# ade-ma/LibRedio

Measured on NVIDIA B200. Metric: Msamples/s cf32 through FIR-decimate+FFT chain, higher is better.
Workload: dtype f32

## Files before the change

libredio_b200/csrc/common.cuh:

```cuda
#pragma once
#include <cuda_runtime.h>
#include <cstdint>
#include <cstdio>
#include <cstdarg>
#include <cstring>
#include <cstdlib>
#include <new>
#include "../../include/libredio_cuda.h"

struct lrc_ctx {
    int          device;
    int          n_sm;
    cudaStream_t stream;
    cudaStream_t copy_stream;
    cudaStream_t out_stream;
    int          numa_node;
    int          numa_nodes;
};

void lrc_set_error(const char *fmt, ...);

#define LRC_CUDA(call)                                                                       \
    do {                                                                                     \
        cudaError_t e__ = (call);                                                            \
        if (e__ != cudaSuccess) {                                                            \
            lrc_set_error("%s:%d %s -> %s", __FILE__, __LINE__, #call, cudaGetErrorString(e__)); \
            return LRC_ERR_CUDA;                                                             \
        }                                                                                    \
    } while (0)

#define LRC_REQUIRE(cond, code, msg)                                                         \
    do {                                                                                     \
        if (!(cond)) {                                                                       \
            lrc_set_error("%s:%d %s", __FILE__, __LINE__, msg);                              \
            return (code);                                                                   \
        }                                                                                    \
    } while (0)

static inline cudaStream_t lrc_stream(const lrc_ctx *ctx, void *s)
{
    return s ? reinterpret_cast<cudaStream_t>(s) : ctx->stream;
}

#define LRC_BIND(ctx)                                                                        \
    do {                                                                                     \
        LRC_REQUIRE((ctx) != nullptr, LRC_ERR_INVALID, "null context");                      \
        LRC_CUDA(cudaSetDevice((ctx)->device));                                              \
    } while (0)

static inline size_t ceil_div(size_t a, size_t b) { return (a + b - 1) / b; }

static inline size_t lrc_grid_mult(const char *env_name, size_t dflt)
{
    const char *e = getenv(env_name);
    if (!e) return dflt;
    const long v = atol(e);
    return v > 0 ? (size_t)v : dflt;
}

#ifdef __CUDACC__

__device__ __forceinline__ uint64_t pk2(float lo, float hi)
{
    uint64_t r;
    asm("mov.b64 %0, {%1, %2};" : "=l"(r) : "f"(lo), "f"(hi));
    return r;
}
__device__ __forceinline__ float2 upk2(uint64_t v)
{
    float2 r;
    asm("mov.b64 {%0, %1}, %2;" : "=f"(r.x), "=f"(r.y) : "l"(v));
    return r;
}
__device__ __forceinline__ float2 add2(float2 a, float2 b)
{
    uint64_t r;
    asm("add.rn.f32x2 %0, %1, %2;" : "=l"(r) : "l"(pk2(a.x, a.y)), "l"(pk2(b.x, b.y)));
    return upk2(r);
}
__device__ __forceinline__ float2 sub2(float2 a, float2 b)
{
    uint64_t r;
    asm("sub.rn.f32x2 %0, %1, %2;" : "=l"(r) : "l"(pk2(a.x, a.y)), "l"(pk2(b.x, b.y)));
    return upk2(r);
}
__device__ __forceinline__ float2 mul2(float2 a, float2 b)
{
    uint64_t r;
    asm("mul.rn.f32x2 %0, %1, %2;" : "=l"(r) : "l"(pk2(a.x, a.y)), "l"(pk2(b.x, b.y)));
    return upk2(r);
}
__device__ __forceinline__ float2 fma2(float2 a, float2 b, float2 c)
{
    uint64_t r;
    asm("fma.rn.f32x2 %0, %1, %2, %3;" : "=l"(r) : "l"(pk2(a.x, a.y)), "l"(pk2(b.x, b.y)), "l"(pk2(c.x, c.y)));
    return upk2(r);
}

__device__ __forceinline__ float2 cmulf(float2 a, float2 b)
{
    return fma2(a, make_float2(b.x, b.x), mul2(make_float2(a.y, a.x), make_float2(-b.y, b.y)));
}
__device__ __forceinline__ float2 cmul_conjb(float2 a, float2 b)
{
    return fma2(a, make_float2(b.x, b.x), mul2(make_float2(a.y, a.x), make_float2(b.y, -b.y)));
}

__device__ __forceinline__ float4 ldg_stream_f4(const float4 *p)
{
    float4 r;
    asm volatile("ld.global.nc.L1::no_allocate.v4.f32 {%0, %1, %2, %3}, [%4];"
                 : "=f"(r.x), "=f"(r.y), "=f"(r.z), "=f"(r.w) : "l"(p));
    return r;
}
__device__ __forceinline__ uint4 ldg_stream_u4(const uint4 *p)
{
    uint4 r;
    asm volatile("ld.global.nc.L1::no_allocate.v4.u32 {%0, %1, %2, %3}, [%4];"
                 : "=r"(r.x), "=r"(r.y), "=r"(r.z), "=r"(r.w) : "l"(p));
    return r;
}
__device__ __forceinline__ void stg_stream_f4(float4 *p, float4 v)
{
    asm volatile("st.global.L1::no_allocate.v4.f32 [%0], {%1, %2, %3, %4};"
                 :: "l"(p), "f"(v.x), "f"(v.y), "f"(v.z), "f"(v.w) : "memory");
}

__device__ __forceinline__ uint32_t smem_u32(const void *p)
{
    return static_cast<uint32_t>(__cvta_generic_to_shared(p));
}

__device__ __forceinline__ void mbar_init(uint64_t *bar, uint32_t count)
{
    asm volatile("mbarrier.init.shared::cta.b64 [%0], %1;" :: "r"(smem_u32(bar)), "r"(count));
}
__device__ __forceinline__ void mbar_fence_init()
{
    asm volatile("fence.mbarrier_init.release.cluster;" ::: "memory");
}
__device__ __forceinline__ void mbar_expect_tx(uint64_t *bar, uint32_t bytes)
{
    asm volatile("mbarrier.arrive.expect_tx.shared::cta.b64 _, [%0], %1;"
                 :: "r"(smem_u32(bar)), "r"(bytes) : "memory");
}
__device__ __forceinline__ void mbar_wait(uint64_t *bar, uint32_t parity)
{
    asm volatile(
        "{\n"
        ".reg .pred p;\n"
        "WAIT_%=:\n"
        "mbarrier.try_wait.parity.shared::cta.b64 p, [%0], %1;\n"
        "@p bra DONE_%=;\n"
        "bra WAIT_%=;\n"
        "DONE_%=:\n"
        "}\n" :: "r"(smem_u32(bar)), "r"(parity) : "memory");
}
__device__ __forceinline__ void tma_load_1d(void *smem_dst, const void *gmem_src, uint32_t bytes,
                                            uint64_t *bar)
{
    asm volatile(
        "cp.async.bulk.shared::cluster.global.mbarrier::complete_tx::bytes [%0], [%1], %2, [%3];"
        :: "r"(smem_u32(smem_dst)), "l"(gmem_src), "r"(bytes), "r"(smem_u32(bar)) : "memory");
}
__device__ __forceinline__ void tma_load_1d_evict_first(void *smem_dst, const void *gmem_src,
                                                        uint32_t bytes, uint64_t *bar)
{
    uint64_t pol;
    asm volatile("createpolicy.fractional.L2::evict_first.b64 %0, 1.0;" : "=l"(pol));
    asm volatile(
        "cp.async.bulk.shared::cluster.global.mbarrier::complete_tx::bytes.L2::cache_hint [%0], [%1], %2, [%3], %4;"
        :: "r"(smem_u32(smem_dst)), "l"(gmem_src), "r"(bytes), "r"(smem_u32(bar)), "l"(pol) : "memory");
}
__device__ __forceinline__ void cp_async4(void *smem_dst, const void *gmem_src, uint32_t src_bytes)
{
    asm volatile("cp.async.ca.shared.global [%0], [%1], 4, %2;" :: "r"(smem_u32(smem_dst)), "l"(gmem_src), "r"(src_bytes) : "memory");
}
__device__ __forceinline__ void cp_async_commit()
{
    asm volatile("cp.async.commit_group;" ::: "memory");
}
template <int N>
__device__ __forceinline__ void cp_async_wait_group()
{
    asm volatile("cp.async.wait_group %0;" :: "n"(N) : "memory");
}
__device__ __forceinline__ void fence_proxy_async()
{
    asm volatile("fence.proxy.async.shared::cta;" ::: "memory");
}
__device__ __forceinline__ void named_bar_sync(int id, int nthreads)
{
    asm volatile("bar.sync %0, %1;" :: "r"(id), "r"(nthreads) : "memory");
}

__device__ __forceinline__ void named_bar_arrive(int id, int nthreads)
{
    asm volatile("bar.arrive %0, %1;" :: "r"(id), "r"(nthreads) : "memory");
}

#endif
```

libredio_b200/csrc/k_chain.cu:

```cuda
#include "fir_core.cuh"
#include "fft_core.cuh"
#include "unpack.cuh"
#include "chain_generic.cuh"
#include <vector>
#include <cmath>

using namespace lrfft;

int    lrc_make_twiddles(int nfft, float2 **d_tw);
int    lrc_log2_exact(int n);
size_t lrc_psd_frames_per_item(size_t k_avg);
int    lrc_psd_ensure_partial(float **d_partial, size_t *cap, size_t need_floats);
int    lrc_psd_reduce(const float *d_partial, float *d_rows, int nfft, size_t ipr, size_t n_rows, float scale,
                      int accumulate, cudaStream_t s);

struct lrc_chain {
    lrc_ctx *ctx;
    int      ntaps, decim, nfft, log2n, window;
    bool     fused;
    bool     fused_generic;
    std::vector<float> taps;
    float2  *d_tw;
    float   *d_win;
    float   *d_partial; size_t partial_cap;
    lrc_fir *fir; lrc_psd *psd;
    float   *d_tmp; size_t tmp_cap;
    float   *d_ring[2]; size_t ring_cap;
    uint8_t *d_ring_u8[2]; size_t ring_u8_cap;
    cudaEvent_t ev_ready[2], ev_free[2];
    float   *d_rows; size_t rows_cap;
    float   *d_u8tmp; size_t u8tmp_cap;
};

template <int NTAPS, int DECIM, int LOG2N, int R>
struct ChainCfg {
    using Tile = FirTile<NTAPS, DECIM, R>;
    using FFT = CtaFFT<LOG2N, false>;
    static constexpr int N = 1 << LOG2N;
    static constexpr int FRAME_ADV = N * DECIM;
    static constexpr int TILE_IN = (N - 1) * DECIM + NTAPS;
    static constexpr int NFIR = (N + R - 1) / R;
    static constexpr int NFIR_T = (NFIR + 31) / 32 * 32;
    static constexpr int NFFT_T = FFT::T;
    static constexpr int NT = NFIR_T + NFFT_T;
    static constexpr int TILE_SAMPLES = (NFIR - 1) * Tile::STEP + Tile::WIN;
    static constexpr uint32_t TMA_BYTES = TILE_IN * 8;
    static constexpr uint32_t RAW_BYTES = TILE_IN * 2;
    static constexpr uint32_t RAW_TMA_BYTES = RAW_BYTES & ~15u;
    static constexpr int RAW_WORDS = (RAW_BYTES + 3) / 4;
    static constexpr int RAW_OFF = (TILE_SAMPLES * 8 - (int)((RAW_BYTES + 15) & ~15u)) & ~15;
    static constexpr int RAW_PER_THREAD = (RAW_WORDS + NFIR_T - 1) / NFIR_T;
    static_assert(RAW_BYTES % 4 == 0, "whole words");
    static_assert((RAW_BYTES - RAW_TMA_BYTES) / 4 <= NFIR_T, "the rest words fall into the last two words of their owners");
    static constexpr int OFF_HAND = TILE_SAMPLES * 8;
    static constexpr int OFF_XCHG = OFF_HAND + FFT::SMEM_CPX * 8;
    static constexpr int OFF_BAR = OFF_XCHG + FFT::SMEM_CPX * 8;
    static constexpr int SMEM_BYTES = OFF_BAR + 16;
    static_assert(TMA_BYTES % 16 == 0 && (FRAME_ADV * 8) % 16 == 0, "TMA alignment");
    static_assert(NFFT_T % 32 == 0, "FFT threads must be whole warps");
};

enum { BAR_FULL = 1, BAR_EMPTY = 2, BAR_TILE = 3, BAR_FFT = 4 };

template <int NTAPS, int DECIM, int LOG2N, int R, bool IS_U8>
__global__ void __launch_bounds__(ChainCfg<NTAPS, DECIM, LOG2N, R>::NT, 2)
chain_kernel(const float2 *__restrict__ in, const float2 *__restrict__ tw, const float *__restrict__ win,
             float *__restrict__ partial, size_t k_avg, size_t fpi, size_t ipr, size_t n_items,
             const __grid_constant__ FirTaps<NTAPS> taps)
{
    using Cfg = ChainCfg<NTAPS, DECIM, LOG2N, R>;
    using Tile = typename Cfg::Tile;
    using FFT = typename Cfg::FFT;
    constexpr int N = Cfg::N, E = FFT::E, T = FFT::T;
    extern __shared__ __align__(128) uint8_t smem[];
    float2 *tile = reinterpret_cast<float2 *>(smem);
    float2 *hand = reinterpret_cast<float2 *>(smem + Cfg::OFF_HAND);
    float2 *xchg = reinterpret_cast<float2 *>(smem + Cfg::OFF_XCHG);
    uint64_t *bar = reinterpret_cast<uint64_t *>(smem + Cfg::OFF_BAR);
    const int tid = threadIdx.x;
    if (tid == 0) { mbar_init(bar, 1); mbar_fence_init(); }
    __syncthreads();
    if ((size_t)blockIdx.x >= n_items) return;

    auto item_range = [&](size_t item, size_t &f0, size_t &f1) {
        const size_t row = item / ipr, c = item % ipr;
        f0 = row * k_avg + c * fpi;
        f1 = f0 + fpi;
        if (f1 > (row + 1) * k_avg) f1 = (row + 1) * k_avg;
    };

    if (tid < Cfg::NFIR_T) {
        uint32_t phase = 0;
        bool first = true;
        size_t item = blockIdx.x, f0, f1;
        item_range(item, f0, f1);
        size_t f = f0;
        const uint8_t *in8 = reinterpret_cast<const uint8_t *>(in);
        uint8_t *raw = smem + Cfg::RAW_OFF;
        auto load_frame = [&](size_t fr) {
            if (IS_U8) {
                mbar_expect_tx(bar, Cfg::RAW_TMA_BYTES);
                tma_load_1d_evict_first(raw, in8 + fr * (size_t)Cfg::FRAME_ADV * 2, Cfg::RAW_TMA_BYTES, bar);
            } else {
                mbar_expect_tx(bar, Cfg::TMA_BYTES);
                tma_load_1d_evict_first(tile, in + fr * Cfg::FRAME_ADV, Cfg::TMA_BYTES, bar);
            }
        };
        if (tid == 0) load_frame(f);
        while (true) {
            if (IS_U8) {
                constexpr int TMA_WORDS = (int)(Cfg::RAW_TMA_BYTES / 4), KL = Cfg::RAW_PER_THREAD;
                uint32_t rest[2] = {0u, 0u};
#pragma unroll
                for (int k = KL - 2; k < KL; ++k) {
                    const int i = tid + k * Cfg::NFIR_T;
                    if (k >= 0 && i >= TMA_WORDS && i < Cfg::RAW_WORDS)
                        rest[k - (KL - 2)] = *reinterpret_cast<const uint32_t *>(in8 + f * (size_t)Cfg::FRAME_ADV * 2 + 4 * (size_t)i);
                }
                mbar_wait(bar, phase);
                uint32_t wv[Cfg::RAW_PER_THREAD];
                const uint32_t *rw = reinterpret_cast<const uint32_t *>(raw);
#pragma unroll
                for (int k = 0; k < KL; ++k) {
                    const int i = tid + k * Cfg::NFIR_T;
                    wv[k] = i < TMA_WORDS ? rw[i] : (k >= KL - 2 ? rest[k - (KL - 2)] : 0u);
                }
                named_bar_sync(BAR_TILE, Cfg::NFIR_T);
                float4 *t4 = reinterpret_cast<float4 *>(tile);
#pragma unroll
                for (int k = 0; k < Cfg::RAW_PER_THREAD; ++k) {
                    const int i = tid + k * Cfg::NFIR_T;
                    if (i < Cfg::RAW_WORDS)
                        t4[i] = make_float4(lr_i2f_byte(wv[k], 0), lr_i2f_byte(wv[k], 1), lr_i2f_byte(wv[k], 2), lr_i2f_byte(wv[k], 3));
                }
                named_bar_sync(BAR_TILE, Cfg::NFIR_T);
            } else {
                mbar_wait(bar, phase);
            }
            phase ^= 1;
            float2 acc[R];
            if (tid < Cfg::NFIR) Tile::run_cf32(tile + (size_t)tid * Tile::STEP, taps, acc);
            size_t nf = f + 1, nitem = item, nf1 = f1;
            if (nf == f1) {
                nitem = item + gridDim.x;
                if (nitem < n_items) item_range(nitem, nf, nf1);
            }
            const bool has_next = nitem < n_items;
            named_bar_sync(BAR_TILE, Cfg::NFIR_T);
            if (tid == 0 && has_next) load_frame(nf);
            if (!first) named_bar_sync(BAR_EMPTY, Cfg::NT);
            first = false;
            if (tid < Cfg::NFIR) {
#pragma unroll
                for (int r = 0; r < R; ++r) {
                    const int o = tid * R + r;
                    if (o < N) hand[FFT::pad(o)] = acc[r];
                }
            }
            __threadfence_block();
            named_bar_arrive(BAR_FULL, Cfg::NT);
            if (!has_next) break;
            item = nitem; f = nf; f1 = nf1;
        }
    } else {
        const int t = tid - Cfg::NFIR_T;
        float w[E], acc[E];
#pragma unroll
        for (int e = 0; e < E; ++e) { w[e] = win[t + e * T]; acc[e] = 0.f; }
        size_t item = blockIdx.x, f0, f1;
        item_range(item, f0, f1);
        size_t f = f0;
        while (true) {
            size_t nf = f + 1, nitem = item, nf1 = f1;
            if (nf == f1) {
                nitem = item + gridDim.x;
                if (nitem < n_items) item_range(nitem, nf, nf1);
            }
            const bool has_next = nitem < n_items;
            named_bar_sync(BAR_FULL, Cfg::NT);
            float2 v[E];
#pragma unroll
            for (int e = 0; e < E; ++e) {
                const float2 x = hand[FFT::pad(t + e * T)];
                v[e] = make_float2(x.x * w[e], x.y * w[e]);
            }
            if (has_next) named_bar_arrive(BAR_EMPTY, Cfg::NT);
            FFT::run(v, xchg, tw, t, SyncNamed{BAR_FFT, T});
#pragma unroll
            for (int e = 0; e < E; ++e) acc[e] = fmaf(v[e].x, v[e].x, fmaf(v[e].y, v[e].y, acc[e]));
            const bool item_done = (f + 1 == f1);
            if (item_done) {
                float *dst = partial + item * N + t;
#pragma unroll
                for (int e = 0; e < E; ++e) { dst[e * T] = acc[e]; acc[e] = 0.f; }
            }
            if (!has_next) break;
            item = nitem; f = nf; f1 = nf1;
        }
    }
}

static const size_t SEG_FRAMES = 400;

extern "C" int lrc_chain_create(lrc_ctx *ctx, const float *h_taps, int ntaps, int decim, int nfft, int window,
                                lrc_chain **out)
{
    LRC_BIND(ctx);
    LRC_REQUIRE(out && h_taps && ntaps >= 1 && decim >= 1, LRC_ERR_INVALID, "lrc_chain_create: bad arguments");
    const int l2 = lrc_log2_exact(nfft);
    if (l2 < 1 || l2 > 13) {
        lrc_set_error("lrc_chain_create: nfft=%d: only powers of two in [2, 8192]", nfft);
        return LRC_ERR_UNSUPPORTED;
    }
    lrc_chain *c = new (std::nothrow) lrc_chain();
    LRC_REQUIRE(c != nullptr, LRC_ERR_NOMEM, "out of host memory");
    c->ctx = ctx; c->ntaps = ntaps; c->decim = decim; c->nfft = nfft; c->log2n = l2; c->window = window;
    c->taps.assign(h_taps, h_taps + ntaps);
    c->fused = (ntaps == 64 && decim == 10 && nfft == 1024);
    c->fused_generic = false;
    if (!c->fused && !getenv("LRC_CHAIN_NO_GENERIC")) {
        c->fused_generic = lrc_chaing_has(ntaps, decim, l2, getenv("LRC_CHAIN_GENERIC_ALL") != nullptr);
    }
    c->d_tw = nullptr; c->d_win = nullptr; c->d_partial = nullptr; c->partial_cap = 0;
    c->fir = nullptr; c->psd = nullptr; c->d_tmp = nullptr; c->tmp_cap = 0;
    c->d_ring[0] = c->d_ring[1] = nullptr; c->ring_cap = 0; c->d_rows = nullptr; c->rows_cap = 0;
    c->d_ring_u8[0] = c->d_ring_u8[1] = nullptr; c->ring_u8_cap = 0;
    c->d_u8tmp = nullptr; c->u8tmp_cap = 0;
    c->ev_ready[0] = c->ev_ready[1] = c->ev_free[0] = c->ev_free[1] = nullptr;
    int rc = lrc_fir_create(ctx, h_taps, ntaps, decim, &c->fir);
    if (!rc) rc = lrc_psd_create(ctx, nfft, window, &c->psd);
    if (!rc) rc = lrc_make_twiddles(nfft, &c->d_tw);
    if (!rc) {
        std::vector<float> w(nfft);
        const double pi = 3.14159265358979323846264338327950288;
        for (int i = 0; i < nfft; ++i)
            w[i] = window == LRC_WINDOW_HANN ? (float)(0.5 - 0.5 * cos(2.0 * pi * i / nfft)) : 1.0f;
        if (cudaMalloc(&c->d_win, sizeof(float) * nfft) != cudaSuccess ||
            cudaMemcpy(c->d_win, w.data(), sizeof(float) * nfft, cudaMemcpyHostToDevice) != cudaSuccess) {
            lrc_set_error("lrc_chain_create: %s", cudaGetErrorString(cudaGetLastError()));
            rc = LRC_ERR_CUDA;
        }
    }
    if (rc) { lrc_chain_destroy(c); return rc; }
    *out = c;
    return LRC_OK;
}

extern "C" int lrc_chain_destroy(lrc_chain *c)
{
    if (!c) return LRC_OK;
    cudaSetDevice(c->ctx->device);
    lrc_fir_destroy(c->fir); lrc_psd_destroy(c->psd);
    cudaFree(c->d_tw); cudaFree(c->d_win); cudaFree(c->d_partial); cudaFree(c->d_tmp);
    cudaFree(c->d_ring[0]); cudaFree(c->d_ring[1]); cudaFree(c->d_rows);
    cudaFree(c->d_ring_u8[0]); cudaFree(c->d_ring_u8[1]); cudaFree(c->d_u8tmp);
    for (int i = 0; i < 2; ++i) {
        if (c->ev_ready[i]) cudaEventDestroy(c->ev_ready[i]);
        if (c->ev_free[i]) cudaEventDestroy(c->ev_free[i]);
    }
    delete c;
    return LRC_OK;
}

extern "C" size_t lrc_chain_frames(const lrc_chain *c, size_t n_in)
{
    if (!c) return 0;
    const size_t tile_in = (size_t)(c->nfft - 1) * c->decim + c->ntaps;
    if (n_in < tile_in) return 0;
    return (n_in - tile_in) / ((size_t)c->nfft * c->decim) + 1;
}

extern "C" int lrc_chain_kind(const lrc_chain *c)
{
    if (!c) return 0;
    return c->fused ? 1 : (c->fused_generic ? 2 : 0);
}

template <bool IS_U8>
static int chain_launch_fused(lrc_chain *c, const void *d_in, size_t k_local, size_t fpi, size_t ipr, size_t n_items, cudaStream_t s)
{
    using Cfg = ChainCfg<64, 10, 10, 7>;
    auto kern = chain_kernel<64, 10, 10, 7, IS_U8>;
    LRC_CUDA(cudaFuncSetAttribute(kern, cudaFuncAttributeMaxDynamicSharedMemorySize, Cfg::SMEM_BYTES));
    int occ = 1;
    LRC_CUDA(cudaOccupancyMaxActiveBlocksPerMultiprocessor(&occ, kern, Cfg::NT, Cfg::SMEM_BYTES));
    if (occ < 1) occ = 1;
    static const size_t gm = lrc_grid_mult("LRC_CHAIN_GRID", 1);
    size_t blocks = (size_t)c->ctx->n_sm * occ * gm;
    if (blocks > n_items) blocks = n_items;
    FirTaps<64> taps;
    for (int i = 0; i < 64; ++i) taps.h[i] = c->taps[i];
    kern<<<(unsigned)blocks, Cfg::NT, Cfg::SMEM_BYTES, s>>>((const float2 *)d_in, c->d_tw, c->d_win, c->d_partial,
                                                           k_local, fpi, ipr, n_items, taps);
    LRC_CUDA(cudaGetLastError());
    return LRC_OK;
}

static int chain_launch(lrc_chain *c, const void *d_in_any, int input_is_u8, size_t rows_local, size_t k_local, float *d_rows,
                        float scale, int accumulate, cudaStream_t s)
{
    const float *d_in = (const float *)d_in_any;
    if (rows_local == 0 || k_local == 0) return LRC_OK;
    const size_t fpi = lrc_psd_frames_per_item(k_local);
    const size_t ipr = ceil_div(k_local, fpi);
    const size_t n_items = rows_local * ipr;
    int rc = lrc_psd_ensure_partial(&c->d_partial, &c->partial_cap, n_items * (size_t)c->nfft);
    if (rc) return rc;
    if (c->fused) {
        rc = input_is_u8 ? chain_launch_fused<true>(c, d_in_any, k_local, fpi, ipr, n_items, s)
                         : chain_launch_fused<false>(c, d_in_any, k_local, fpi, ipr, n_items, s);
        if (rc) return rc;
        return lrc_psd_reduce(c->d_partial, d_rows, c->nfft, ipr, rows_local, scale, accumulate, s);
    }
    LRC_REQUIRE(!input_is_u8, LRC_ERR_INVALID, "chain_launch: u8 input without a fused instance");
    if (c->fused_generic) {
        chaing::Args a;
        a.in = (const float2 *)d_in_any; a.tw = c->d_tw; a.win = c->d_win; a.taps = c->taps.data(); a.partial = c->d_partial;
        a.k_avg = k_local; a.fpi = fpi; a.ipr = ipr; a.n_items = n_items; a.ntaps = c->ntaps; a.n_sm = c->ctx->n_sm; a.stream = s;
        const int grc = lrc_chaing_launch(a, c->decim, c->log2n);
        if (grc > 0) return grc;
        if (grc == 0) return lrc_psd_reduce(c->d_partial, d_rows, c->nfft, ipr, rows_local, scale, accumulate, s);
    }
    const size_t n_frames = rows_local * k_local;
    const size_t n_dec = n_frames * (size_t)c->nfft;
    const size_t n_in = (n_dec - 1) * (size_t)c->decim + c->ntaps;
    if (c->tmp_cap < n_dec * 2 + (size_t)c->nfft * rows_local) {
        cudaFree(c->d_tmp); c->d_tmp = nullptr; c->tmp_cap = 0;
        LRC_CUDA(cudaMalloc(&c->d_tmp, (n_dec * 2 + (size_t)c->nfft * rows_local) * sizeof(float)));
        c->tmp_cap = n_dec * 2 + (size_t)c->nfft * rows_local;
    }
    rc = lrc_fir_run_cf32(c->fir, d_in, 1, n_in, n_in, c->d_tmp, n_dec, s);
    if (rc) return rc;
    float *rows_tmp = c->d_tmp + n_dec * 2;
    rc = lrc_psd_run(c->psd, c->d_tmp, n_frames, k_local, rows_tmp, s);
    if (rc) return rc;
    return lrc_psd_reduce(rows_tmp, d_rows, c->nfft, 1, rows_local, scale * (float)k_local, accumulate, s);
}

extern "C" int lrc_chain_run(lrc_chain *c, const float *d_in, size_t n_in, size_t k_avg, float *d_rows,
                             size_t *n_rows, void *stream)
{
    LRC_REQUIRE(c != nullptr, LRC_ERR_INVALID, "null plan");
    LRC_BIND(c->ctx);
    LRC_REQUIRE(k_avg >= 1, LRC_ERR_INVALID, "lrc_chain_run: k_avg must be >= 1");
    const size_t rows = lrc_chain_frames(c, n_in) / k_avg;
    if (n_rows) *n_rows = rows;
    if (rows == 0) return LRC_OK;
    LRC_REQUIRE(d_in && d_rows, LRC_ERR_INVALID, "lrc_chain_run: null buffer");
    LRC_REQUIRE(((uintptr_t)d_in & 15) == 0, LRC_ERR_INVALID, "lrc_chain_run: input must be 16-byte aligned");
    return chain_launch(c, d_in, 0, rows, k_avg, d_rows, 1.0f / (float)k_avg, 0, lrc_stream(c->ctx, stream));
}

extern "C" int lrc_chain_run_u8(lrc_chain *c, const uint8_t *d_iq, size_t n_in, size_t k_avg, float *d_rows,
                                size_t *n_rows, void *stream)
{
    LRC_REQUIRE(c != nullptr, LRC_ERR_INVALID, "null plan");
    LRC_BIND(c->ctx);
    LRC_REQUIRE(k_avg >= 1, LRC_ERR_INVALID, "lrc_chain_run_u8: k_avg must be >= 1");
    const size_t rows = lrc_chain_frames(c, n_in) / k_avg;
    if (n_rows) *n_rows = rows;
    if (rows == 0) return LRC_OK;
    LRC_REQUIRE(d_iq && d_rows, LRC_ERR_INVALID, "lrc_chain_run_u8: null buffer");
    cudaStream_t s = lrc_stream(c->ctx, stream);
    if (c->fused) {
        LRC_REQUIRE(((uintptr_t)d_iq & 15) == 0, LRC_ERR_INVALID, "lrc_chain_run_u8: input must be 16-byte aligned");
        return chain_launch(c, d_iq, 1, rows, k_avg, d_rows, 1.0f / (float)k_avg, 0, s);
    }
    const size_t need = (rows * k_avg - 1) * (size_t)c->nfft * c->decim + (size_t)(c->nfft - 1) * c->decim + c->ntaps;
    if (c->u8tmp_cap < need) {
        cudaFree(c->d_u8tmp); c->d_u8tmp = nullptr; c->u8tmp_cap = 0;
        LRC_CUDA(cudaMalloc(&c->d_u8tmp, need * sizeof(float2)));
        c->u8tmp_cap = need;
    }
    const int urc = lrc_unpack_u8_cf32(c->ctx, d_iq, need * 2, c->d_u8tmp, s);
    if (urc) return urc;
    return chain_launch(c, c->d_u8tmp, 0, rows, k_avg, d_rows, 1.0f / (float)k_avg, 0, s);
}

static int chain_run_host_impl(lrc_chain *c, const void *h_in_any, int input_is_u8, size_t n_in, size_t k_avg,
                               float *h_rows, size_t *n_rows)
{
    const float *h_in = (const float *)h_in_any;
    const uint8_t *h_in_u8 = (const uint8_t *)h_in_any;
    LRC_REQUIRE(c != nullptr, LRC_ERR_INVALID, "null plan");
    LRC_BIND(c->ctx);
    LRC_REQUIRE(k_avg >= 1, LRC_ERR_INVALID, "lrc_chain_run_host: k_avg must be >= 1");
    const size_t rows = lrc_chain_frames(c, n_in) / k_avg;
    if (n_rows) *n_rows = rows;
    if (rows == 0) return LRC_OK;
    LRC_REQUIRE(h_in && h_rows, LRC_ERR_INVALID, "lrc_chain_run_host: null buffer");
    const size_t adv = (size_t)c->nfft * c->decim;
    const size_t tile_in = (size_t)(c->nfft - 1) * c->decim + c->ntaps;
    const size_t tail = (size_t)c->ntaps > (size_t)c->decim ? (size_t)c->ntaps - c->decim : 0;
    const bool slice_rows = k_avg > SEG_FRAMES;
    const size_t seg_frames = slice_rows ? SEG_FRAMES / 16 * 16 : (SEG_FRAMES / k_avg) * k_avg;
    const size_t slot_samples = seg_frames * adv + tail + 8;
    const bool direct_u8 = input_is_u8 && c->fused;
    if (!direct_u8 && c->ring_cap < slot_samples) {
        for (int i = 0; i < 2; ++i) { cudaFree(c->d_ring[i]); c->d_ring[i] = nullptr; }
        c->ring_cap = 0;
        for (int i = 0; i < 2; ++i) LRC_CUDA(cudaMalloc(&c->d_ring[i], slot_samples * sizeof(float2)));
        c->ring_cap = slot_samples;
    }
    if (input_is_u8 && c->ring_u8_cap < slot_samples) {
        for (int i = 0; i < 2; ++i) { cudaFree(c->d_ring_u8[i]); c->d_ring_u8[i] = nullptr; }
        c->ring_u8_cap = 0;
        for (int i = 0; i < 2; ++i) LRC_CUDA(cudaMalloc(&c->d_ring_u8[i], slot_samples * 2));
        c->ring_u8_cap = slot_samples;
    }
    if (c->rows_cap < rows * (size_t)c->nfft) {
        cudaFree(c->d_rows); c->d_rows = nullptr; c->rows_cap = 0;
        LRC_CUDA(cudaMalloc(&c->d_rows, rows * (size_t)c->nfft * sizeof(float)));
        c->rows_cap = rows * (size_t)c->nfft;
    }
    for (int i = 0; i < 2; ++i) {
        if (!c->ev_ready[i]) LRC_CUDA(cudaEventCreateWithFlags(&c->ev_ready[i], cudaEventDisableTiming));
        if (!c->ev_free[i]) LRC_CUDA(cudaEventCreateWithFlags(&c->ev_free[i], cudaEventDisableTiming));
    }
    cudaStream_t cs = c->ctx->copy_stream, ks = c->ctx->stream;
    const size_t total_frames = rows * k_avg;
    const float scale = 1.0f / (float)k_avg;
    size_t seg = 0;
    for (size_t f = 0; f < total_frames; ++seg) {
        size_t nfr = seg_frames;
        if (slice_rows) {
            const size_t row_end = (f / k_avg + 1) * k_avg;
            if (f + nfr > row_end) nfr = row_end - f;
        }
        if (f + nfr > total_frames) nfr = total_frames - f;
        const int b = (int)(seg & 1);
        const size_t ns = (nfr - 1) * adv + tile_in;
        if (seg >= 2) LRC_CUDA(cudaStreamWaitEvent(cs, c->ev_free[b], 0));
        if (input_is_u8)
            LRC_CUDA(cudaMemcpyAsync(c->d_ring_u8[b], h_in_u8 + 2 * f * adv, ns * 2, cudaMemcpyHostToDevice, cs));
        else
            LRC_CUDA(cudaMemcpyAsync(c->d_ring[b], h_in + 2 * f * adv, ns * sizeof(float2), cudaMemcpyHostToDevice, cs));
        LRC_CUDA(cudaEventRecord(c->ev_ready[b], cs));
        LRC_CUDA(cudaStreamWaitEvent(ks, c->ev_ready[b], 0));
        if (input_is_u8 && !direct_u8) {
            const int urc = lrc_unpack_u8_cf32(c->ctx, c->d_ring_u8[b], ns * 2, c->d_ring[b], ks);
            if (urc) return urc;
        }
        const void *seg_in = direct_u8 ? (const void *)c->d_ring_u8[b] : (const void *)c->d_ring[b];
        int rc;
        if (slice_rows) {
            const size_t row = f / k_avg;
            rc = chain_launch(c, seg_in, direct_u8, 1, nfr, c->d_rows + row * c->nfft, scale, (f % k_avg) != 0, ks);
        } else {
            rc = chain_launch(c, seg_in, direct_u8, nfr / k_avg, k_avg, c->d_rows + (f / k_avg) * c->nfft, scale, 0, ks);
        }
        if (rc) return rc;
        LRC_CUDA(cudaEventRecord(c->ev_free[b], ks));
        f += nfr;
    }
    LRC_CUDA(cudaMemcpyAsync(h_rows, c->d_rows, rows * (size_t)c->nfft * sizeof(float), cudaMemcpyDeviceToHost, ks));
    LRC_CUDA(cudaStreamSynchronize(ks));
    return LRC_OK;
}

extern "C" int lrc_chain_run_host(lrc_chain *c, const float *h_in, size_t n_in, size_t k_avg, float *h_rows,
                                  size_t *n_rows)
{
    return chain_run_host_impl(c, h_in, 0, n_in, k_avg, h_rows, n_rows);
}

extern "C" int lrc_chain_run_host_u8(lrc_chain *c, const uint8_t *h_iq, size_t n_in, size_t k_avg, float *h_rows,
                                     size_t *n_rows)
{
    return chain_run_host_impl(c, h_iq, 1, n_in, k_avg, h_rows, n_rows);
}
```

Baseline: 860,600.

## Add warp-specialized TMA ring-buffer chain kernel for cf32 FIR+FFT path

Adds a new fused chain kernel for the ntaps=64, decim=10, nfft=1024 cf32 case. It uses warp specialization: one producer thread streams frame tiles into a two-slot shared-memory ring with TMA bulk loads and full/empty mbarriers. FIR warps compute into a handoff buffer, and FFT warps window, transform and accumulate power, with named barriers handing frames between the stages. The goal is to overlap global loads, FIR and FFT across frames instead of running them in sequence within a CTA. The cost is one CTA per SM with heavy shared-memory use, and the named-barrier handoff may serialize the FIR and FFT stages.

```diff
diff --git a/libredio_b200/csrc/common.cuh b/libredio_b200/csrc/common.cuh
--- a/libredio_b200/csrc/common.cuh
+++ b/libredio_b200/csrc/common.cuh
@@ -144,6 +144,10 @@
     asm volatile("mbarrier.arrive.expect_tx.shared::cta.b64 _, [%0], %1;"
                  :: "r"(smem_u32(bar)), "r"(bytes) : "memory");
 }
+__device__ __forceinline__ void mbar_arrive(uint64_t *bar)
+{
+    asm volatile("mbarrier.arrive.shared::cta.b64 _, [%0];" :: "r"(smem_u32(bar)) : "memory");
+}
 __device__ __forceinline__ void mbar_wait(uint64_t *bar, uint32_t parity)
 {
     asm volatile(
diff --git a/libredio_b200/csrc/k_chain.cu b/libredio_b200/csrc/k_chain.cu
--- a/libredio_b200/csrc/k_chain.cu
+++ b/libredio_b200/csrc/k_chain.cu
@@ -18,6 +18,7 @@
     lrc_ctx *ctx;
     int      ntaps, decim, nfft, log2n, window;
     bool     fused;
+    bool     ring;
     bool     fused_generic;
     std::vector<float> taps;
     float2  *d_tw;
@@ -200,6 +201,142 @@
     }
 }
 
+template <int NTAPS, int DECIM, int LOG2N, int R>
+struct RingCfg {
+    using Tile = FirTile<NTAPS, DECIM, R>;
+    using FFT = CtaFFT<LOG2N, false>;
+    static constexpr int N = 1 << LOG2N, NBUF = 2;
+    static constexpr int FRAME_ADV = N * DECIM;
+    static constexpr int TILE_IN = (N - 1) * DECIM + NTAPS;
+    static constexpr int NFIR = (N + R - 1) / R;
+    static constexpr int NFIR_T = (NFIR + 31) / 32 * 32;
+    static constexpr int PROD = NFIR_T;
+    static constexpr int FFT0 = PROD + 32;
+    static constexpr int NT = FFT0 + FFT::T;
+    static constexpr int NHAND = NFIR_T + FFT::T;
+    static constexpr int TILE_SAMPLES = (NFIR - 1) * Tile::STEP + Tile::WIN;
+    static constexpr int SLOT_BYTES = (TILE_SAMPLES * 8 + 127) / 128 * 128;
+    static constexpr uint32_t TMA_BYTES = TILE_IN * 8;
+    static constexpr int OFF_HAND = NBUF * SLOT_BYTES;
+    static constexpr int OFF_XCHG = OFF_HAND + FFT::SMEM_CPX * 8;
+    static constexpr int OFF_BAR = OFF_XCHG + FFT::SMEM_CPX * 8;
+    static constexpr int SMEM_BYTES = OFF_BAR + 2 * NBUF * 8;
+    static_assert(R % 2 == 1 && (Tile::STEP * 8 / 16) % 2 == 1, "thread windows an odd multiple of 16 bytes apart: conflict-free LDS.128");
+    static_assert(TMA_BYTES % 16 == 0 && (FRAME_ADV * 8) % 16 == 0, "TMA alignment");
+    static_assert(SMEM_BYTES <= 227 * 1024, "one CTA per SM");
+};
+
+struct FrameCursor {
+    size_t k_avg, fpi, ipr, n_items;
+    size_t item, f, f1;
+    bool ok;
+    __device__ __forceinline__ void item_range()
+    {
+        const size_t row = item / ipr, c = item % ipr;
+        f = row * k_avg + c * fpi;
+        f1 = f + fpi;
+        if (f1 > (row + 1) * k_avg) f1 = (row + 1) * k_avg;
+    }
+    __device__ __forceinline__ FrameCursor(size_t k_avg_, size_t fpi_, size_t ipr_, size_t n_items_)
+        : k_avg(k_avg_), fpi(fpi_), ipr(ipr_), n_items(n_items_), item(blockIdx.x), ok(true) { item_range(); }
+    __device__ __forceinline__ void advance()
+    {
+        if (++f < f1) return;
+        item += gridDim.x;
+        if (item < n_items) item_range();
+        else ok = false;
+    }
+};
+
+template <int NTAPS, int DECIM, int LOG2N, int R>
+__global__ void __launch_bounds__(RingCfg<NTAPS, DECIM, LOG2N, R>::NT, 1)
+chain_ring_kernel(const float2 *__restrict__ in, const float2 *__restrict__ tw, const float *__restrict__ win,
+                  float *__restrict__ partial, size_t k_avg, size_t fpi, size_t ipr, size_t n_items,
+                  const __grid_constant__ FirTaps<NTAPS> taps)
+{
+    using Cfg = RingCfg<NTAPS, DECIM, LOG2N, R>;
+    using Tile = typename Cfg::Tile;
+    using FFT = typename Cfg::FFT;
+    constexpr int N = Cfg::N, E = FFT::E, T = FFT::T, NBUF = Cfg::NBUF;
+    extern __shared__ __align__(128) uint8_t smem[];
+    float2 *hand = reinterpret_cast<float2 *>(smem + Cfg::OFF_HAND);
+    float2 *xchg = reinterpret_cast<float2 *>(smem + Cfg::OFF_XCHG);
+    uint64_t *full = reinterpret_cast<uint64_t *>(smem + Cfg::OFF_BAR), *empty = full + NBUF;
+    auto slot = [&](int b) { return reinterpret_cast<float2 *>(smem + (size_t)b * Cfg::SLOT_BYTES); };
+    const int tid = threadIdx.x;
+    if (tid == 0) {
+#pragma unroll
+        for (int b = 0; b < NBUF; ++b) { mbar_init(full + b, 1); mbar_init(empty + b, Cfg::NFIR_T / 32); }
+        mbar_fence_init();
+    }
+    __syncthreads();
+    if ((size_t)blockIdx.x >= n_items) return;
+
+    if (tid < Cfg::NFIR_T) {
+        FrameCursor cur(k_avg, fpi, ipr, n_items);
+        for (uint32_t q = 0;; ++q) {
+            const int b = (int)(q % NBUF);
+            mbar_wait(full + b, (q / NBUF) & 1u);
+            float2 acc[R];
+            if (tid < Cfg::NFIR) Tile::run_cf32(slot(b) + (size_t)tid * Tile::STEP, taps, acc);
+            __syncwarp();
+            if ((tid & 31) == 0) mbar_arrive(empty + b);
+            if (q > 0) named_bar_sync(BAR_EMPTY, Cfg::NHAND);
+            if (tid < Cfg::NFIR) {
+#pragma unroll
+                for (int r = 0; r < R; ++r) {
+                    const int o = tid * R + r;
+                    if (o < N) hand[FFT::pad(o)] = acc[r];
+                }
+            }
+            __threadfence_block();
+            named_bar_arrive(BAR_FULL, Cfg::NHAND);
+            cur.advance();
+            if (!cur.ok) break;
+        }
+    } else if (tid < Cfg::FFT0) {
+        if (tid == Cfg::PROD) {
+            FrameCursor ld(k_avg, fpi, ipr, n_items);
+            for (uint32_t q = 0; ld.ok; ++q) {
+                const int b = (int)(q % NBUF);
+                if (q >= NBUF) mbar_wait(empty + b, (q / NBUF - 1) & 1u);
+                mbar_expect_tx(full + b, Cfg::TMA_BYTES);
+                tma_load_1d_evict_first(slot(b), in + ld.f * Cfg::FRAME_ADV, Cfg::TMA_BYTES, full + b);
+                ld.advance();
+            }
+        }
+    } else {
+        const int t = tid - Cfg::FFT0;
+        float w[E], acc[E];
+#pragma unroll
+        for (int e = 0; e < E; ++e) { w[e] = win[t + e * T]; acc[e] = 0.f; }
+        FrameCursor cur(k_avg, fpi, ipr, n_items);
+        while (true) {
+            const size_t item = cur.item;
+            const bool item_done = cur.f + 1 == cur.f1;
+            cur.advance();
+            const bool has_next = cur.ok;
+            named_bar_sync(BAR_FULL, Cfg::NHAND);
+            float2 v[E];
+#pragma unroll
+            for (int e = 0; e < E; ++e) {
+                const float2 x = hand[FFT::pad(t + e * T)];
+                v[e] = make_float2(x.x * w[e], x.y * w[e]);
+            }
+            if (has_next) named_bar_arrive(BAR_EMPTY, Cfg::NHAND);
+            FFT::run(v, xchg, tw, t, SyncNamed{BAR_FFT, T});
+#pragma unroll
+            for (int e = 0; e < E; ++e) acc[e] = fmaf(v[e].x, v[e].x, fmaf(v[e].y, v[e].y, acc[e]));
+            if (item_done) {
+                float *dst = partial + item * N + t;
+#pragma unroll
+                for (int e = 0; e < E; ++e) { dst[e * T] = acc[e]; acc[e] = 0.f; }
+            }
+            if (!has_next) break;
+        }
+    }
+}
+
 static const size_t SEG_FRAMES = 400;
 
 extern "C" int lrc_chain_create(lrc_ctx *ctx, const float *h_taps, int ntaps, int decim, int nfft, int window,
@@ -218,6 +355,8 @@
     c->taps.assign(h_taps, h_taps + ntaps);
     c->fused = (ntaps == 64 && decim == 10 && nfft == 1024);
     c->fused_generic = false;
+    const char *ring_env = getenv("LRC_CHAIN_RING");
+    c->ring = c->fused && !(ring_env && strcmp(ring_env, "0") == 0);
     if (!c->fused && !getenv("LRC_CHAIN_NO_GENERIC")) {
         c->fused_generic = lrc_chaing_has(ntaps, decim, l2, getenv("LRC_CHAIN_GENERIC_ALL") != nullptr);
     }
@@ -276,11 +415,10 @@
     return c->fused ? 1 : (c->fused_generic ? 2 : 0);
 }
 
-template <bool IS_U8>
-static int chain_launch_fused(lrc_chain *c, const void *d_in, size_t k_local, size_t fpi, size_t ipr, size_t n_items, cudaStream_t s)
-{
-    using Cfg = ChainCfg<64, 10, 10, 7>;
-    auto kern = chain_kernel<64, 10, 10, 7, IS_U8>;
+template <class Cfg, class Kern>
+static int chain_launch_instance(lrc_chain *c, Kern kern, const void *d_in, size_t k_local, size_t fpi, size_t ipr, size_t n_items,
+                                 cudaStream_t s)
+{
     LRC_CUDA(cudaFuncSetAttribute(kern, cudaFuncAttributeMaxDynamicSharedMemorySize, Cfg::SMEM_BYTES));
     int occ = 1;
     LRC_CUDA(cudaOccupancyMaxActiveBlocksPerMultiprocessor(&occ, kern, Cfg::NT, Cfg::SMEM_BYTES));
@@ -294,6 +432,14 @@
                                                            k_local, fpi, ipr, n_items, taps);
     LRC_CUDA(cudaGetLastError());
     return LRC_OK;
+}
+
+template <bool IS_U8>
+static int chain_launch_fused(lrc_chain *c, const void *d_in, size_t k_local, size_t fpi, size_t ipr, size_t n_items, cudaStream_t s)
+{
+    if (!IS_U8 && c->ring)
+        return chain_launch_instance<RingCfg<64, 10, 10, 7>>(c, chain_ring_kernel<64, 10, 10, 7>, d_in, k_local, fpi, ipr, n_items, s);
+    return chain_launch_instance<ChainCfg<64, 10, 10, 7>>(c, chain_kernel<64, 10, 10, 7, IS_U8>, d_in, k_local, fpi, ipr, n_items, s);
 }
 
 static int chain_launch(lrc_chain *c, const void *d_in_any, int input_is_u8, size_t rows_local, size_t k_local, float *d_rows,
```

Result: faster. 878,400 (median of 6 runs) (+2.1%).
